# hupe1980/vecgo

Measured on AMD Instinct MI355X. Metric: QPS at recall@10≥0.95, 1M×768 HNSW+PQ; PQ-ADC HBM GB/s vs peak, higher is better.
Workload: dtype f32; 1 GPU; flat_exact_l2_1Mx768_top10 (BASELINE configs[1]): MFMA GEMM nomination + exact re-score + proof; operating_point=flat_exact, rows=1000000, dim=768, k=10, parallelism=1 GPU

## Files before the change

vecgo_amd/csrc/k_flat.hip:

```cpp
#include <algorithm>

#include "vg_device.hpp"
#include "vg_exact.hpp"
#include "vg_cand_replay.hpp"
#include "vg_flat_gemm.hpp"
#include "vg_internal.hpp"
#include "vg_nominate.hpp"
#include "vg_search.hpp"

namespace vg {

struct GemmOperands {
    const float *a, *b;
    int64_t n;
    int dim_words;
    const float *norms;
    bool bf16, dma;
};
struct NomCall {
    hipStream_t st;
    bool dot;
    GemmOperands ops;
    int64_t cnt;
    const uint8_t *mask;
    int64_t mask_stride;
    unsigned ucnt() const { return static_cast<unsigned>(cnt); }
};
struct GemmArgs {
    const NomCall &c;
    const float *queries;
    float *scores = nullptr;
    int tile_stride = 1;
    int64_t out_cols = 0;
    const float *thr = nullptr;
    int thr_stride = 0, thr_off = 0;
    int *counts = nullptr;
    uint64_t *cand = nullptr;
    int cap = 0;
    int cus = 256;
    int *counts_wide = nullptr;
    int skip_stride = 0;
    bool split = false;
    bool screen = false;
    const uint32_t *tile_active = nullptr;

    explicit GemmArgs(const NomCall &call) : c(call), queries(call.ops.a) {}
    static GemmArgs sample(const NomCall &c, float *sc, int stride, int64_t cols)
    {
        GemmArgs a(c);
        a.scores = sc, a.tile_stride = stride, a.out_cols = cols;
        return a;
    }
    static GemmArgs append(const NomCall &c, const float *thr, int sel_k, int *counts, uint64_t *cand, int cap)
    {
        GemmArgs a(c);
        a.thr = thr, a.thr_stride = sel_k, a.thr_off = sel_k - 1, a.counts = counts, a.cand = cand, a.cap = cap;
        return a;
    }
    GemmArgs &wide(int *lines, int compute_units) { return counts_wide = lines, cus = compute_units, *this; }
    GemmArgs &skipping(int stride) { return skip_stride = stride, *this; }
    GemmArgs &split_tile(const uint32_t *image) { return queries = reinterpret_cast<const float *>(image), split = true, *this; }
    GemmArgs &sample_tile(const uint32_t *hi_image) { return split_tile(hi_image); }
    GemmArgs &screen_tile(const uint32_t *hi_image) { return split_tile(hi_image), screen = true, *this; }
    GemmArgs &retry(const uint32_t *active) { return tile_active = active, *this; }
};
constexpr int kCountLine = 32;
static bool gemm_runs_split(bool fused, bool bf16, bool dma, int64_t nq, int dim, int cap, int thr_stride)
{
    return fused && !bf16 && dma && nq > kGemmBM && dim % kGemmBK == 0 && nq * static_cast<int64_t>(cap) < (int64_t(1) << 31) &&
           thr_stride < 65536 && !hook(kHookFlatNoSplit);
}
static float split_gemm_eps(bool dot, int dim)
{
    const float m = static_cast<float>(3 * dim + 16) * 5.9604645e-8f;
    return dot ? 1.5001f * 1.52587890625e-5f + 2.52f * m : 3.0002f * 1.52587890625e-5f + 4.03f * m;
}
static float screen_gemm_eps(bool dot, int dim)
{
    const float m = static_cast<float>(dim + 16) * 5.9604645e-8f;
    return dot ? 0.00390625f + 7.62939453125e-6f + 2.52f * m : 0.0078125f + 1.52587890625e-5f + 4.03f * m;
}
float bf16_filter_eps(bool dot) { return (dot ? 0.00390625f : 0.0078125f) * 1.02f; }
static bool gemm_skips_sample(bool dma, int64_t nq, bool bf16, bool split = false)
{
    if (bf16 || split || hook(kHookFlatRescoreSample)) return false;
    return !(dma && nq <= 3 * kG32BM && !hook(kHookFlatNoSmallTile));
}
__global__ void counts_narrow_kernel(const int *__restrict__ wide, int64_t nq, int *__restrict__ counts)
{
    const int64_t q = static_cast<int64_t>(blockIdx.x) * blockDim.x + threadIdx.x;
    if (q < nq) counts[q] = wide[q * kCountLine];
}

template <class Kern, class... Args>
static int32_t launch_lds(Kern kern, dim3 grid, dim3 threads, size_t lds, hipStream_t st, Args... args)
{
    VG_HIP(hipFuncSetAttribute(reinterpret_cast<const void *>(kern), hipFuncAttributeMaxDynamicSharedMemorySize, static_cast<int>(lds)));
    if (grid.x != 0) VG_LAUNCH(kern, grid, threads, lds, st, args...);
    return VG_OK;
}
template <bool DOT, int M, bool BF16, class F>
static int32_t with_g32_tile(int rb, F f)
{
    constexpr int kMost = BF16 ? 4 : 3;
    if (rb <= 1) return f(flat_gemm_dma32_kernel<DOT, M, 1, BF16>, g32_lds_bytes<1>());
    if (rb == 2) return f(flat_gemm_dma32_kernel<DOT, M, 2, BF16>, g32_lds_bytes<2>());
    if (rb == 3) return f(flat_gemm_dma32_kernel<DOT, M, 3, BF16>, g32_lds_bytes<3>());
    return f(flat_gemm_dma32_kernel<DOT, M, kMost, BF16>, g32_lds_bytes<kMost>());
}

template <bool DOT, int MODE>
static int32_t launch_gemm_t(const GemmArgs &a)
{
    const NomCall &c = a.c;
    const bool dma = c.ops.dma, bf16 = c.ops.bf16;
    const hipStream_t st = c.st;
    const int skip = MODE == 2 ? a.skip_stride : 0;
    VG_CHECK(skip == 0 || (skip > 1 && gemm_skips_sample(dma, c.cnt, bf16, a.split)), VG_ERR_INVALID_ARG, "launch_gemm: skip_stride on a kernel without it");
    const int64_t mt = (c.cnt + kGemmBM - 1) / kGemmBM, nt = (c.ops.n + kGemmBN - 1) / kGemmBN;
    const int64_t tiles = skip ? nt - gemm_skip_sampled_tiles(nt, skip) : (nt + a.tile_stride - 1) / a.tile_stride;
    const dim3 grid(static_cast<unsigned>(mt * ((tiles + 7) / 8) * 8)), threads(kGemmThreads);
    auto big_grid = [&](int64_t bnt ) {
        const int64_t bmt = (c.cnt + kBigBM - 1) / kBigBM;
        const int64_t slots = bmt * ((bnt + 7) / 8) * 8, per_cu = std::max(a.cus / 8, 1) * 8;
        return dim3(static_cast<unsigned>(std::min(slots, per_cu)));
    };
    auto launch_big = [&](auto kern, size_t lds, auto... extra) -> int32_t {
        if (a.counts_wide && !a.tile_active) VG_HIP(hipMemsetAsync(a.counts_wide, 0, sizeof(int) * static_cast<size_t>(c.cnt) * kCountLine, st));
        VG_TRY(launch_lds(kern, big_grid((c.ops.n + kBigBN - 1) / kBigBN), dim3(kBigThreads), lds, st, a.queries, c.cnt, c.ops.b, c.ops.n,
                          c.ops.dim_words, c.ops.norms, a.thr, a.thr_stride, a.thr_off, a.counts_wide ? a.counts_wide : a.counts, a.cand, a.cap, c.mask,
                          c.mask_stride, a.counts_wide ? kCountLine : 1, extra...));
        if (a.counts_wide)
            VG_LAUNCH(counts_narrow_kernel, dim3(static_cast<unsigned>((c.cnt + 255) / 256)), dim3(256), 0, st, a.counts_wide, c.cnt, a.counts);
        return VG_OK;
    };
    auto launch_tile = [&](auto kern, dim3 blocks, size_t lds, auto... last) -> int32_t {
        return launch_lds(kern, blocks, threads, lds, st, a.queries, c.cnt, c.ops.b, c.ops.n, c.ops.dim_words, c.ops.norms, a.scores, a.tile_stride, a.out_cols, a.thr,
                          a.thr_stride, a.thr_off, a.counts, a.cand, a.cap, c.mask, c.mask_stride, last...);
    };
    auto launch_128 = [&](auto kern, size_t lds, int last) { return launch_tile(kern, grid, lds, last); };
    auto launch_g32 = [&](auto kern, size_t lds) { return launch_tile(kern, dim3(static_cast<unsigned>(tiles)), lds); };
    constexpr int M = MODE == 0 ? 1 : MODE;
    const int rb = static_cast<int>((c.cnt + kG32BM - 1) / kG32BM);
    if constexpr (MODE == 1) {
        if (a.split) {
            VG_CHECK(!bf16 && gemm_runs_split(true, false, dma, c.cnt, c.ops.dim_words, 0, 0), VG_ERR_INVALID_ARG, "launch_gemm: sample tile on a call without it");
            return launch_lds(flat_gemm_sample_big_kernel<DOT, 3>, big_grid((tiles + 1) / 2), dim3(kBigThreads), big_lds_bytes<3, true>(), st, a.queries, c.cnt,
                              c.ops.b, c.ops.n, c.ops.dim_words, c.ops.norms, a.scores, a.tile_stride, a.out_cols, c.mask, c.mask_stride);
        }
    }
    if (MODE == 2 && a.split) {
        VG_CHECK(!bf16 && gemm_runs_split(true, false, dma, c.cnt, c.ops.dim_words, a.cap, a.thr_stride), VG_ERR_INVALID_ARG, "launch_gemm: split tile on a call without it");
        if (a.screen) return launch_big(flat_gemm_screen_big_kernel<DOT, 3>, big_lds_bytes<3, true>());
        VG_CHECK(!a.tile_active || (c.cnt <= 32 * kBigBM && a.counts_wide), VG_ERR_INVALID_ARG, "launch_gemm: tile_active is one word, with wide counters");
        note_flat_split_launch();
        return launch_big(flat_gemm_split_big_kernel<DOT, 3>, big_lds_bytes<3>(), a.tile_active);
    }
    if (skip && tiles == 0) return VG_OK;
    if (bf16) {
        if (c.cnt <= 4 * kG32BM && !hook(kHookFlatNoSmallTile)) return with_g32_tile<DOT, M, true>(rb, launch_g32);
        if (MODE == 2 && c.cnt > kGemmBM && c.cnt * static_cast<int64_t>(a.cap) < (int64_t(1) << 31) && a.thr_stride < 65536 &&
            !hook(kHookFlatNoBigTile)) {
            const bool two = hook(kHookFlatBigTile2);
            auto kern = two ? flat_gemm_bf16_big_kernel<DOT, 2> : hook(kHookFlatBigEarlyB) ? flat_gemm_bf16_big_kernel<DOT, 3, 512> : flat_gemm_bf16_big_kernel<DOT, 3>;
            return launch_big(kern, two ? big_lds_bytes<2>() : big_lds_bytes<3>());
        }
        return launch_128(flat_gemm_dma_kernel<DOT, M, 0, true>, kDmaLdsBytes, 0);
    }
    if (dma && MODE != 0 && c.cnt <= 3 * kG32BM && !hook(kHookFlatNoSmallTile)) return with_g32_tile<DOT, M, false>(rb, launch_g32);
    if (dma) return launch_128(flat_gemm_dma_kernel<DOT, MODE>, kDmaLdsBytes, skip);
    return launch_128(flat_gemm_kernel<DOT, MODE>, kGemmLdsBytes, skip);
}

template <int MODE>
static int32_t launch_gemm(const GemmArgs &a)
{
    return a.c.dot ? launch_gemm_t<true, MODE>(a) : launch_gemm_t<false, MODE>(a);
}

__global__ void f32_to_bf16_pad_kernel(const float *__restrict__ src, int64_t rows, int dim, int dim_pad, uint16_t *__restrict__ dst)
{
    const int64_t i = static_cast<int64_t>(blockIdx.x) * blockDim.x + threadIdx.x;
    if (i >= rows * dim_pad) return;
    const int64_t r = i / dim_pad;
    const int j = static_cast<int>(i - r * dim_pad);
    const uint32_t u = j < dim ? __float_as_uint(src[r * dim + j]) : 0u;
    uint16_t v;
    if ((u & 0x7F800000u) == 0x7F800000u && (u & 0x007FFFFFu) != 0)
        v = static_cast<uint16_t>((u >> 16) | 0x0040u);
    else
        v = static_cast<uint16_t>((u + 0x7FFFu + ((u >> 16) & 1u)) >> 16);
    dst[i] = v;
}

static int64_t flat_hi_image_rows(int64_t rows) { return (rows + kBigBM - 1) / kBigBM * kBigBM; }
__global__ void flat_split_queries_kernel(const float *__restrict__ src, int64_t rows, int dim, uint32_t *__restrict__ dst,
                                          uint32_t *__restrict__ hi_dst)
{
    const int64_t i = static_cast<int64_t>(blockIdx.x) * blockDim.x + threadIdx.x;
    const int half = dim / 2;
    const int64_t r = i / half;
    if (r >= (rows + kBigBM - 1) / kBigBM * kBigBM) return;
    const int64_t rs = r < rows ? r : rows - 1;
    const int p = static_cast<int>(i - r * half), s = p >> 4, w = p & 15;
    const float2 v = *reinterpret_cast<const float2 *>(src + rs * dim + 32 * s + 2 * w);
    uint32_t hi, lo;
    split2_bf16(v.x, v.y, hi, lo);
    if (r < rows) {
        dst[r * dim + 32 * s + w] = hi;
        dst[r * dim + 32 * s + 16 + w] = lo;
    }
    const int R = static_cast<int>(r & (kBigBM - 1));
    hi_dst[((r / kBigBM) * (dim / 32) + s) * (kBigBM * 16) + R * 16 + (((w >> 2) ^ ((R >> 2) & 3)) << 2) + (w & 3)] = hi;
}

__global__ __launch_bounds__(256) void flat_todo_kernel(const int *__restrict__ flags, const int *__restrict__ always,
                                                        int cnt, int *__restrict__ todo,
                                                        unsigned long long *__restrict__ stats, const int *__restrict__ counts)
{
    __shared__ int part[256];
    __shared__ unsigned long long appended[256];
    const int tid = threadIdx.x;
    const int per = (cnt + 255) / 256;
    const int lo = tid * per < cnt ? tid * per : cnt, hi = lo + per < cnt ? lo + per : cnt;
    if (!flags) {
        if (tid == 0) atomicAdd(&stats[0], static_cast<unsigned long long>(cnt));
        return;
    }
    const bool all = *always != 0;
    int mine = 0;
    unsigned long long app = 0;
    for (int i = lo; i < hi; i++) {
        mine += (all || flags[i] != 0);
        if (counts) app += static_cast<unsigned long long>(counts[i]);
    }
    part[tid] = mine;
    appended[tid] = app;
    __syncthreads();
    if (tid == 0) {
        int run = 0;
        app = 0;
        for (int t = 0; t < 256; t++) {
            const int c = part[t];
            part[t] = run;
// ... 171 lines not shown
        for (int64_t c = wave; c < chunks; c += kSelWaves) {
            float4 v[4];
#pragma unroll
            for (int u = 0; u < 4; u++) v[u] = row4[c * 256 + u * 64 + lane];
#pragma unroll
            for (int u = 0; u < 4; u++) {
                const int64_t i = a0 + c * 1024 + (u * 64 + lane) * 4;
                const float vals[4] = {v[u].x, v[u].y, v[u].z, v[u].w};
                float mn = fminf(fminf(vals[0], vals[1]), fminf(vals[2], vals[3]));
                if (!__ballot(make_key(mn, 0u, false) < tk.tau)) continue;
#pragma unroll
                for (int e = 0; e < 4; e++)
                    tk.offer(make_key(vals[e], static_cast<uint32_t>(i + e), false), lane);
            }
        }
    }
    {
        const int64_t head_end = (a0 < r1 && a1 > a0) ? a0 : r1;
        for (int64_t i0 = r0 + wave * 64; i0 < head_end; i0 += kSelThreads) {
            const int64_t i = i0 + lane;
            tk.offer(i < head_end ? make_key(row[i], static_cast<uint32_t>(i), false) : kKeyMax, lane);
        }
        const int64_t tail_begin = (a0 < r1 && a1 > a0) ? a1 : r1;
        for (int64_t i0 = tail_begin + wave * 64; i0 < r1; i0 += kSelThreads) {
            const int64_t i = i0 + lane;
            tk.offer(i < r1 ? make_key(row[i], static_cast<uint32_t>(i), false) : kKeyMax, lane);
        }
    }
    wg_rank_merge<kSelWaves>(tk, lists, valid, wave, lane, tid, kc,
                             partial + (q * slices + s) * kc);
}

template <bool DOT>
__global__ __launch_bounds__(256) void flat_verify_kernel(
    const float *__restrict__ base, int64_t n, int dim, const float *__restrict__ queries,
    const float *__restrict__ norms_max , const uint32_t *__restrict__ cand_ids,
    const float *__restrict__ cand_scores, int kc, int k, uint32_t *__restrict__ ids,
    float *__restrict__ scores, int *fallback, const float *__restrict__ thr, int thr_stride,
    int thr_off, const int *__restrict__ counts, int cap, float eps_extra, const int *only)
{
    __shared__ uint64_t keys[64];
    const Sub16 sub = Sub16::make(threadIdx.x);
    const int64_t q = blockIdx.x;
    if (only && only[q] == 0) return;
    const float *qv = queries + q * dim;
    for (int c = threadIdx.x >> 4; c < kc; c += 16) {
        const uint32_t id = cand_ids[q * kc + c];
        uint64_t key = kKeyMax;
        if (id != VG_INVALID_ID) {
            const float v = exact_pair16<DOT, kPair>(base + static_cast<int64_t>(id) * dim, qv, dim, sub);
            key = make_key(v, id, DOT);
        }
        if ((threadIdx.x & 15) == 0) keys[c] = key;
    }
    __syncthreads();
    if (threadIdx.x >= 64) return;
    const int lane = threadIdx.x;
    WaveTopK tk;
    tk.init(k);
    tk.offer(lane < kc ? keys[lane] : kKeyMax, lane);
    float qn = 0.0f;
    for (int j = lane; j < dim; j += 64) qn = __builtin_fmaf(qv[j], qv[j], qn);
    for (int off = 32; off > 0; off >>= 1) qn += __shfl_xor(qn, off);
    const uint64_t kth = readlane_u64(tk.list, k - 1);
    bool ok = true;
    float tau;
    bool have_all;
    if (thr) {
        const float tq = thr[q * thr_stride + thr_off];
        const int cnt = counts[q];
        if (cnt > cap) ok = false;
        tau = cnt > kc ? fminf(tq, cand_scores[q * kc + (kc - 1)]) : tq;
        have_all = (tq == INFINITY) && cnt <= kc;
    } else {
        tau = cand_scores[q * kc + (kc - 1)];
        have_all = (n <= kc);
    }
    if (ok && !have_all) {
        const float xmax = norms_max[0];
        const float eps = (4.0f * (static_cast<float>(dim) * 5.9604645e-8f) + eps_extra) * (qn + xmax) + 1e-30f;
        if (tau == INFINITY) {
            ok = true;
        } else if (kth == kKeyMax) {
            ok = false;
        } else if (DOT) {
            const float dk = key_score(kth, true);
            ok = dk > (-tau) + eps;
        } else {
            const float dk = key_score(kth, false);
            ok = dk < (tau + qn) - eps;
        }
    }
    if (lane < k) {
        const uint64_t e = tk.list;
        ids[q * k + lane] = e == kKeyMax ? VG_INVALID_ID : key_row(e);
        scores[q * k + lane] = e == kKeyMax ? (DOT ? -INFINITY : INFINITY) : key_score(e, DOT);
    }
    if (lane == 0) fallback[q] = ok ? 0 : 1;
}

template <bool DOT>
__global__ __launch_bounds__(256) void flat_verify_all_kernel(
    const float *__restrict__ base, int dim, const float *__restrict__ queries,
    const float *__restrict__ norms_max , const uint64_t *__restrict__ cand, const int *__restrict__ counts,
    int cap, int k, uint32_t *__restrict__ ids, float *__restrict__ scores, int *__restrict__ fallback,
    const float *__restrict__ thr, int thr_stride, int thr_off, float eps_extra)
{
    __shared__ uint64_t lists[4 * 64];
    __shared__ int valid[4];
    __shared__ uint64_t best[64];
    const Sub16 sub = Sub16::make(threadIdx.x);
    const int64_t q = blockIdx.x;
    const int tid = threadIdx.x, lane = tid & 63, wave = tid >> 6;
    const float *qv = queries + q * dim;
    const int total = counts[q];
    const int cnt = total < cap ? total : cap;
    WaveTopK tk;
    tk.init(k);
    for (int c0 = wave * 4; c0 < cnt; c0 += 16) {
        const int c = c0 + (lane >> 4);
        uint64_t key = kKeyMax;
        if (c < cnt) {
            const uint32_t id = key_row(cand[q * cap + c]);
            const float v = exact_pair16<DOT, kPair>(base + static_cast<int64_t>(id) * dim, qv, dim, sub);
            if ((lane & 15) == 0) key = make_key(v, id, DOT);
        }
        tk.offer(key, lane);
    }
    wg_rank_merge<4>(tk, lists, valid, wave, lane, tid, k, best);
    __syncthreads();
    if (tid >= 64) return;
// ... 96 lines not shown
        const uint64_t floor_key = min_keys ? min_keys[q] : 0;
        const uint8_t *mq = mask ? mask + q * mask_stride : nullptr;
        WaveTopK tk;
        tk.init(k);
        for (int64_t i0 = r0 + wave * 4; i0 < r1; i0 += 16) {
            const int64_t i = i0 + (lane >> 4);
            uint64_t key = kKeyMax;
            if (i < r1 && mask_bit(mq, i)) {
                const float v = exact_pair16<DOT, kPair>(base + i * dim, qv, dim, sub);
                if ((lane & 15) == 0) {
                    key = make_key(v, static_cast<uint32_t>(i), DOT);
                    if (min_keys && key <= floor_key) key = kKeyMax;
                }
            }
            tk.offer(key, lane);
        }
        wg_rank_merge<4>(tk, lists, valid, wave, lane, tid, k, out);
        __syncthreads();
    }
}

constexpr int kScanQB = 8;
constexpr int kGemmMaxK = 48;
constexpr int kFlatMaxK = 512;
constexpr int kScreenMaxK = 16;
static bool gemm_runs_screen(bool split, int k)
{
    return split && !hook(kHookFlatNoScreen) && k <= (hook(kHookFlatScreenFail) ? kGemmMaxK : kScreenMaxK);
}
static bool sample_runs_big(bool split, bool use_sample)
{
    return split && use_sample && !hook(kHookFlatF32Sample);
}
constexpr int kScanMaxBatch = 4;
template <bool DOT>
__global__ __launch_bounds__(256) void flat_scan_mq_kernel(const float *__restrict__ base, int64_t n, int dim,
                                                           const float *__restrict__ queries, int nq, int slices,
                                                           int k, uint64_t *__restrict__ partial)
{
    extern __shared__ float qlds[];
    uint64_t *lists = reinterpret_cast<uint64_t *>(qlds + static_cast<size_t>(kScanQB) * dim);
    int *valid = reinterpret_cast<int *>(lists + 4 * 64);
    const int s = blockIdx.x;
    const int tid = threadIdx.x, lane = tid & 63, wave = tid >> 6;
    for (int t = tid; t < nq * dim; t += 256) qlds[t] = queries[t];
    __syncthreads();
    const Sub16 sub = Sub16::make(tid);
    const int nblk = dim >> 6;
    const int64_t r0 = n * s / slices, r1 = n * (s + 1) / slices;
    WaveTopK tk[kScanQB];
#pragma unroll
    for (int qi = 0; qi < kScanQB; qi++) tk[qi].init(k);
    for (int64_t i0 = r0 + wave * 4; i0 < r1; i0 += 16) {
        const int64_t i = i0 + (lane >> 4);
        const bool live = i < r1;
        const float *row = base + (live ? i : r1 - 1) * dim;
        float4 rr[16];
        const float4 *r4 = reinterpret_cast<const float4 *>(row) + sub.f4;
#pragma unroll
        for (int e = 0; e < 16; e++)
            if (e < nblk) rr[e] = load_stream(r4 + e * 16);
#pragma unroll
        for (int qi = 0; qi < kScanQB; qi++) {
            if (qi < nq) {
                const float v = exact_rowregs16<DOT>(rr, nblk, row, qlds + static_cast<size_t>(qi) * dim, dim, sub);
                uint64_t key = kKeyMax;
// ... 107 lines not shown
}
static int32_t sample_thresholds(const NomCall &c, const NomScratch &s, int stride, int sel_k, float *thr, bool sampled, const uint32_t *image = nullptr,
                                 int cus = 0)
{
    if (!sampled) {
        VG_LAUNCH(fill_f32_kernel, dim3(static_cast<unsigned>((c.cnt * sel_k + 255) / 256)), dim3(256), 0, c.st, thr, c.cnt * sel_k, INFINITY);
        return VG_OK;
    }
    GemmArgs a = GemmArgs::sample(c, s.sc, stride, s.cols);
    if (image) a.sample_tile(image).wide(nullptr, cus);
    VG_TRY(launch_gemm<1>(a));
    return select_thresholds(s, c.cnt, sel_k, s.sid, thr, c.st);
}
static int32_t launch_flat_pick(const ProbeNominated &nom, int64_t cnt, const int *only, hipStream_t st)
{
    VG_LAUNCH(flat_pick_kernel, dim3(static_cast<unsigned>(cnt)), dim3(256), 0, st, nom.cand, nom.counts, nom.cap, kFlatKc, nom.cand_id, nom.cand_sc, only);
    return VG_OK;
}
static int32_t launch_flat_verify(bool dot, int k, const vg_index *idx, const float *queries, int64_t cnt, const ProbeNominated &nom,
                                  float eps_extra, uint32_t *ids, float *scores, int *fail, const int *only, hipStream_t st)
{
    return with_metric(dot, [&](auto dot_c) -> int32_t {
        constexpr bool DOT = decltype(dot_c)::value;
        const dim3 grid(static_cast<unsigned>(cnt)), threads(256);
        if (nom.thr && k > 64)
            VG_LAUNCH(flat_verify_sort_kernel<DOT>, grid, threads, sizeof(uint64_t) * static_cast<size_t>(nom.cap), st, idx->d_vectors, idx->dim, queries,
                      idx->d_norm_max, nom.cand, nom.counts, nom.cap, k, ids, scores, fail, nom.thr, nom.sel_k, nom.sel_k - 1, eps_extra);
        else if (nom.thr && k > kGemmMaxK)
            VG_LAUNCH(flat_verify_all_kernel<DOT>, grid, threads, 0, st, idx->d_vectors, idx->dim, queries, idx->d_norm_max, nom.cand, nom.counts,
                      nom.cap, k, ids, scores, fail, nom.thr, nom.sel_k, nom.sel_k - 1, eps_extra);
        else
            VG_LAUNCH(flat_verify_kernel<DOT>, grid, threads, 0, st, idx->d_vectors, idx->n, idx->dim, queries, idx->d_norm_max, nom.cand_id,
                      nom.cand_sc, kFlatKc, k, ids, scores, fail, nom.thr, nom.sel_k, nom.sel_k - 1, nom.counts, nom.cap, eps_extra, only);
        return VG_OK;
    });
}

struct FlatCall {
    vg_index *idx;
    int k;
    hipStream_t st;
    bool dot;
    const float *q;
    int64_t nq;
    const uint8_t *mask;
    int64_t mask_stride;
    uint32_t *oid;
    float *osc;
    int64_t n = idx->n;
    int dim = idx->dim;
    FlatCall range(int64_t q0, int64_t cnt) const
    {
        FlatCall r = *this;
        r.q += q0 * dim, r.nq = cnt, r.oid += q0 * k, r.osc += q0 * k;
        if (mask) r.mask += q0 * mask_stride;
        return r;
    }
    NomCall nom() const { return {st, dot, fp32_operands(idx, q, !hook(kHookFlatNoDma)), nq, mask, mask_stride}; }
};
constexpr int kFlatCap = 4096;
constexpr int kFlatSampleStride = 64;
static int exact_slices(int64_t n) { return static_cast<int>(std::min<int64_t>(256, std::max<int64_t>(1, n / 64))); }
struct FlatScratch : NomScratch {
    bool fused;
    bool use_sample;
    bool bf16;
// ... 74 lines not shown
    int *flags = ar.get<int>(i_flags), *todo = ar.get<int>(i_todo);
    uint64_t *fpartial = ar.get<uint64_t>(i_fpartial);
    VG_HIP(hipMemsetAsync(flags, 0, sizeof(int) * static_cast<size_t>(qc), call.st));
    VG_HIP(hipMemsetAsync(flags + qc, 1, sizeof(int), call.st));
    for (int64_t q0 = 0; q0 < call.nq; q0 += qc) {
        const FlatCall c = call.range(q0, std::min(qc, call.nq - q0));
        VG_TRY(launch_flat_todo(flags, flags + qc, static_cast<int>(c.nq), todo, c.idx->d_flat_stats, c.st));
        VG_TRY(launch_flat_exact(c, todo, ex_slices, c.k, fpartial, nullptr));
        VG_TRY(launch_topk_merge(fpartial, c.nq, ex_slices, c.k, c.dot, c.oid, c.osc, c.st));
    }
    return VG_OK;
}

static int32_t flat_unfused_chunk(const FlatCall &c, const FlatScratch &s)
{
    const NomCall nc = c.nom();
    {
        ProfScope prof(c.idx->ctx, "flat_gemm", c.st);
        VG_TRY(launch_gemm<0>(GemmArgs::sample(nc, s.sc, 1, c.n)));
    }
    {
        ProfScope prof(c.idx->ctx, "flat_select", c.st);
        VG_TRY(launch_flat_select(s, c.nq, kFlatKc, c.st));
    }
    VG_TRY(launch_topk_merge(s.partial, c.nq, s.slices, kFlatKc, false, s.nom.cand_id, s.nom.cand_sc, c.st));
    ProbeNominated nom = s.nom;
    nom.thr = nullptr;
    return launch_flat_verify(c.dot, c.k, c.idx, c.q, c.nq, nom, 0.0f, c.oid, c.osc, s.flags, nullptr, c.st);
}

static int32_t flat_screen_retry(const FlatCall &c, const NomCall &nc, const FlatScratch &s)
{
    const ProbeNominated &nom = s.nom;
    VG_LAUNCH(flat_retry_prepare_kernel, dim3(1), dim3(kBigBM), 0, c.st, s.flags, hook(kHookFlatScreenFail), static_cast<int>(c.nq), nom.thr,
              nom.sel_k, nom.sel_k - 1, nom.counts, s.counts_wide, s.tile_active, c.idx->d_flat_stats);
    {
        ProfScope prof(c.idx->ctx, "flat_retry", c.st);
        VG_TRY(launch_gemm<2>(GemmArgs::append(nc, nom.thr, nom.sel_k, nom.counts, nom.cand, nom.cap)
                                  .wide(s.counts_wide, c.idx->ctx->compute_units)
                                  .split_tile(reinterpret_cast<const uint32_t *>(s.qbf))
                                  .retry(s.tile_active)));
    }
    VG_TRY(launch_flat_pick(nom, c.nq, s.flags, c.st));
    return launch_flat_verify(c.dot, c.k, c.idx, c.q, c.nq, nom, split_gemm_eps(c.dot, c.dim), c.oid, c.osc, s.flags, s.flags, c.st);
}

static int32_t flat_fused_chunk(const FlatCall &c, const FlatScratch &s)
{
    const vg_index *idx = c.idx;
    const ProbeNominated &nom = s.nom;
    NomCall nc = c.nom();
    const bool split = gemm_runs_split(true, s.bf16, nc.ops.dma, c.nq, c.dim, nom.cap, nom.sel_k);
    const bool screen = gemm_runs_screen(split, c.k);
    const float eps_extra = screen ? screen_gemm_eps(c.dot, c.dim) : split ? split_gemm_eps(c.dot, c.dim) : s.bf16 ? bf16_filter_eps(c.dot) : 0.0f;
    if (s.bf16) VG_TRY(gemm_operands(c.q, c.nq, c.dim, c.n, idx->d_norms, idx->d_vectors_bf16, idx->vectors_bf16_dim, s.qbf, c.st, &nc.ops));
    if (split)
        VG_LAUNCH(flat_split_queries_kernel, dim3(static_cast<unsigned>((flat_hi_image_rows(c.nq) * (c.dim / 2) + 255) / 256)), dim3(256), 0, c.st, c.q,
                  c.nq, c.dim, reinterpret_cast<uint32_t *>(s.qbf), s.qhi);
    VG_TRY(sample_thresholds(nc, s, kFlatSampleStride, nom.sel_k, nom.thr, s.use_sample, sample_runs_big(split, s.use_sample) ? s.qhi : nullptr,
                             idx->ctx->compute_units));
    if (s.bf16 || split) VG_LAUNCH(flat_thr_cap_kernel, dim3(nc.ucnt()), dim3(64), 0, c.st, nom.thr, nom.sel_k, c.q, c.dim, idx->d_norm_max);
    const bool once = s.use_sample && gemm_skips_sample(nc.ops.dma, c.nq, s.bf16, split);
    if (!once) VG_HIP(hipMemsetAsync(nom.counts, 0, sizeof(int) * static_cast<size_t>(c.nq), c.st));
    {
        ProfScope prof(idx->ctx, "flat_gemm", c.st);
        if (once)
            VG_LAUNCH(flat_sample_append_kernel, dim3(nc.ucnt()), dim3(kSampleAppendThreads), 0, c.st, s.sc, s.cols, kFlatSampleStride, nom.thr,
                      nom.sel_k, nom.sel_k - 1, nom.counts, nom.cand, nom.cap);
        GemmArgs a = GemmArgs::append(nc, nom.thr, nom.sel_k, nom.counts, nom.cand, nom.cap);
        a.wide(s.bf16 || split ? s.counts_wide : nullptr, idx->ctx->compute_units).skipping(once ? kFlatSampleStride : 0);
        if (screen)
            a.screen_tile(s.qhi);
        else if (split)
            a.split_tile(reinterpret_cast<const uint32_t *>(s.qbf));
        VG_TRY(launch_gemm<2>(a));
    }
    if (c.k <= kGemmMaxK) VG_TRY(launch_flat_pick(nom, c.nq, nullptr, c.st));
    VG_TRY(launch_flat_verify(c.dot, c.k, idx, c.q, c.nq, nom, eps_extra, c.oid, c.osc, s.flags, nullptr, c.st));
    return screen ? flat_screen_retry(c, nc, s) : VG_OK;
}

static void flat_debug_counts(const FlatCall &c, int64_t q0, const FlatScratch &s)
{
    std::vector<int> hf(c.nq), hc(c.nq);
    (void)hipMemcpyAsync(hf.data(), s.flags, sizeof(int) * c.nq, hipMemcpyDeviceToHost, c.st);
    (void)hipMemcpyAsync(hc.data(), s.nom.counts, sizeof(int) * c.nq, hipMemcpyDeviceToHost, c.st);
    (void)hipStreamSynchronize(c.st);
    int64_t nf = 0, csum = 0, cmax = 0;
    for (int f : hf) nf += f != 0;
    for (int n : hc) { csum += n; cmax = std::max<int64_t>(cmax, n); }
    fprintf(stderr, "[vg_search_flat] chunk q0=%lld cnt=%lld: %lld queries failed the proof; "
            "appended candidates avg %.1f max %lld\n", (long long)q0, (long long)c.nq, (long long)nf,
            s.fused ? double(csum) / c.nq : 0.0, (long long)(s.fused ? cmax : 0));
}

static int32_t flat_fallback_pages(const FlatCall &c, const FlatScratch &s)
{
    const int *always = s.flags + s.qc;
    const dim3 grid(static_cast<unsigned>(c.nq));
    for (int off = 0; off < c.k; off += 64) {
        const int kk = std::min(64, c.k - off);
        VG_TRY(launch_flat_exact(c, s.todo, s.ex_slices, kk, s.fpartial, off ? s.min_keys : nullptr));
        VG_TRY(launch_topk_merge(s.fpartial, c.nq, s.ex_slices, kk, c.dot, s.fid, s.fsc, c.st, s.flags, always));
        if (c.k <= 64)
            VG_LAUNCH(flat_patch_kernel, grid, dim3(64), 0, c.st, s.flags, always, c.k, s.fid, s.fsc, c.oid, c.osc);
        else
            VG_LAUNCH(flat_page_patch_kernel, grid, dim3(64), 0, c.st, s.flags, always, c.k, off, kk, c.dot, s.fid, s.fsc, c.oid, c.osc, s.min_keys);
    }
    return VG_OK;
}

// ... 298 lines not shown
```

vecgo_amd/csrc/vg_api.hip:

```cpp
#include "vg_internal.hpp"

namespace vg {

static thread_local std::string g_last_error;

void set_error(const char *fmt, ...)
{
    char buf[512];
    va_list ap;
    va_start(ap, fmt);
    vsnprintf(buf, sizeof buf, fmt, ap);
    va_end(ap);
    g_last_error = buf;
}

bool is_device_ptr(const void *p)
{
    if (!p) return false;
    hipPointerAttribute_t a;
    hipError_t e = hipPointerGetAttributes(&a, p);
    (void)hipGetLastError();
    if (e != hipSuccess) return false;
    return a.type == hipMemoryTypeDevice || a.type == hipMemoryTypeManaged;
}
// ... 266 lines not shown
    if (idx->d_flat_stats) (void)hipFree(idx->d_flat_stats);
    if (idx->d_vectors_bf16) (void)hipFree(idx->d_vectors_bf16);
    if (idx->d_rq_tiles) (void)hipFree(idx->d_rq_tiles);
    if (idx->d_rq_norms) (void)hipFree(idx->d_rq_norms);
    for (uint32_t **a : {&idx->d_hnsw_l0, &idx->d_hnsw_slot, &idx->d_hnsw_adj}) vg::drop_device(a);
    for (float **a : {&idx->d_hnsw_l0_dist, &idx->d_hnsw_l0_cdist, &idx->d_hnsw_adj_cdist}) vg::drop_device(a);
    vg::drop_device(&idx->d_hnsw_tomb);
    vg::drop_device(&idx->d_hnsw_level_off);
    if (idx->d_vamana) (void)hipFree(idx->d_vamana);
    if (idx->d_pq_rows) (void)hipFree(idx->d_pq_rows);
    if (idx->d_rq_rows) (void)hipFree(idx->d_rq_rows);
    if (idx->d_sq_tiles) (void)hipFree(idx->d_sq_tiles);
    (void)vg::nom_free(idx->sq_nom, idx->ctx->stream);
    (void)vg::nom_free(idx->pq_nom, idx->ctx->stream);
    if (idx->d_int4_rows) (void)hipFree(idx->d_int4_rows);
    if (idx->d_centroids) (void)hipFree(idx->d_centroids);
    if (idx->d_part_off) (void)hipFree(idx->d_part_off);
    delete idx;
    return VG_OK;
}

#include <atomic>
namespace vg {
static std::atomic<int> g_hooks[kHookCount];
static std::once_flag g_hooks_once;
static const char *const kHookNames[kHookCount] = {"VG_FLAT_NO_SMALL_TILE", "VG_FLAT_UNFUSED", "VG_FLAT_NO_SCAN",
                                                   "VG_FLAT_FORCE_EXACT", "VG_FLAT_NO_DMA", "VG_FLAT_DEBUG",
                                                   "VG_PROBE_NO_GROUP", "VG_ADC_BIGK_EXHAUSTIVE", "VG_BUILD_DEBUG",
                                                   "VG_KM_NO_MFMA", "VG_KM_LIST_ALL", "VG_KM_BF16", "VG_KM_NO_BF16", "VG_BRUTE_NO_FLAT", "VG_PQ_NO_MFMA",
                                                   "VG_PQ_LIST_ALL", "VG_PQ_FP32_MFMA", "VG_PROBE_NO_GEMM", "VG_FLAT_NO_BIG_TILE",
                                                   "VG_FLAT_BIG_TILE_2", "VG_FLAT_BIG_EARLY_B", "VG_PQ_NOM_ALWAYS", "VG_KM_NO_RANGES", "VG_NO_CAND_REPLAY",
                                                   "VG_VAMANA_SMALL_SCRATCH", "VG_FLAT_RESCORE_SAMPLE", "VG_PTHR_FORCE_HIST",
                                                   "VG_WALK_SMALL_SCRATCH", "VG_FLAT_NO_SPLIT", "VG_FLAT_NO_SCREEN", "VG_FLAT_SCREEN_FAIL",
                                                   "VG_FLAT_F32_SAMPLE", "VG_PREFILTER_SMALL_SCRATCH"};
static void hooks_from_env()
{
    for (int h = 0; h < kHookCount; h++) {
        const char *e = getenv(kHookNames[h]);
        g_hooks[h].store(e && e[0] == '1' ? 1 : 0, std::memory_order_relaxed);
    }
}
bool hook(Hook h)
{
    std::call_once(g_hooks_once, hooks_from_env);
    return g_hooks[h].load(std::memory_order_relaxed) != 0;
}
}

VG_API int32_t vg_debug_set_hook(const char *name, int32_t on)
{
    VG_CHECK(name, VG_ERR_INVALID_ARG, "vg_debug_set_hook: NULL name");
    std::call_once(vg::g_hooks_once, vg::hooks_from_env);
    for (int h = 0; h < vg::kHookCount; h++)
        if (std::strcmp(name, vg::kHookNames[h]) == 0) {
            vg::g_hooks[h].store(on ? 1 : 0, std::memory_order_relaxed);
            return VG_OK;
        }
    vg::set_error("vg_debug_set_hook: unknown hook %s", name);
    return VG_ERR_INVALID_ARG;
}
```

vecgo_amd/csrc/vg_internal.hpp:

```cpp
#pragma once

#include <hip/hip_runtime.h>

#include <algorithm>
#include <atomic>
#include <cstdarg>
#include <cstdint>
#include <cstdio>
#include <cstdlib>
#include <cstring>
#include <mutex>
#include <string>
#include <vector>

#include "../../include/vecgo_hip.h"

struct vg_index;

#define VG_API extern "C" __attribute__((visibility("default")))

namespace vg {

void set_error(const char *fmt, ...);

// ... 40 lines not shown
    kHookFlatNoSmallTile,
    kHookFlatUnfused,
    kHookFlatNoScan,
    kHookFlatForceExact,
    kHookFlatNoDma,
    kHookFlatDebug,
    kHookProbeNoGroup,
    kHookAdcBigkExhaustive,
    kHookBuildDebug,
    kHookKmNoMfma,
    kHookKmListAll,
    kHookKmBf16,
    kHookKmNoBf16,
    kHookBruteNoFlat,
    kHookPqNoMfma,
    kHookPqListAll,
    kHookPqFp32Mfma,
    kHookProbeNoGemm,
    kHookFlatNoBigTile,
    kHookFlatBigTile2,
    kHookFlatBigEarlyB,
    kHookPqNomAlways,
    kHookKmNoRanges,
    kHookNoCandReplay,
    kHookVamanaSmallScratch,
    kHookFlatRescoreSample,
    kHookPthrForceHist,
    kHookWalkSmallScratch,
    kHookFlatNoSplit,
    kHookFlatNoScreen,
    kHookFlatScreenFail,
    kHookFlatF32Sample,
    kHookPrefilterSmallScratch,
    kHookCount
};
bool hook(Hook h);

int32_t scratch_alloc(void **out, size_t bytes, hipStream_t s);
int32_t append_row_norms(vg_index *idx, int64_t from, int64_t to, hipStream_t st);
int32_t append_bf16_rows(vg_index *idx, int64_t from, int64_t to, hipStream_t st);
void scratch_free(void *p);
void scratch_trim(int device);

}

struct vg_prof_record {
    const char *name;
    hipEvent_t start, stop;
};

struct vg_arena {
    char *base = nullptr;
    size_t cap = 0;
};

struct vg_ctx {
    int device = 0;
    std::mutex arena_mu;
    std::vector<std::pair<hipStream_t, vg_arena>> arenas;
    hipStream_t stream = nullptr;
    int compute_units = 0;
    int64_t hbm_bytes = 0;
    char arch[64] = {0};
    bool profiling = false;
    std::mutex prof_mu;
    std::vector<vg_prof_record> prof;
// ... 373 lines not shown
```

Before: 509,200 queries/s.

## Fuse candidate pick, exact verify and retry-prepare into one kernel

Adds a flat_pick_verify kernel that merges each query's appended candidates into a top-64 list, re-scores them exactly and runs the proof in one launch. This replaces the separate pick, verify and retry-prepare kernels. The wide per-line counters are zeroed inside the query-split kernel instead of by a memset, and the narrowing kernel is skipped because the fused kernel reads the wide counters directly. The aim is to remove several small launches and memsets plus an intermediate candidate round-trip, at the cost of a larger per-query workgroup kernel and more complex counter state handling.

Result: no change. 510,400 queries/s, median of 3 (+0.2%).

```diff
diff --git a/vecgo_amd/csrc/k_flat.hip b/vecgo_amd/csrc/k_flat.hip
--- a/vecgo_amd/csrc/k_flat.hip
+++ b/vecgo_amd/csrc/k_flat.hip
@@ -39,6 +39,7 @@
     int cap = 0;
     int cus = 256;
     int *counts_wide = nullptr;
+    bool wide_zeroed = false, wide_stays = false;
     int skip_stride = 0;
     bool split = false;
     bool screen = false;
@@ -58,6 +59,7 @@
         return a;
     }
     GemmArgs &wide(int *lines, int compute_units) { return counts_wide = lines, cus = compute_units, *this; }
+    GemmArgs &wide_kept(bool zeroed, bool stays) { return wide_zeroed = zeroed, wide_stays = stays, *this; }
     GemmArgs &skipping(int stride) { return skip_stride = stride, *this; }
     GemmArgs &split_tile(const uint32_t *image) { return queries = reinterpret_cast<const float *>(image), split = true, *this; }
     GemmArgs &sample_tile(const uint32_t *hi_image) { return split_tile(hi_image); }
@@ -69,6 +71,10 @@
 {
     return fused && !bf16 && dma && nq > kGemmBM && dim % kGemmBK == 0 && nq * static_cast<int64_t>(cap) < (int64_t(1) << 31) &&
            thr_stride < 65536 && !hook(kHookFlatNoSplit);
+}
+static bool gemm_runs_big_bf16(int64_t nq, int cap, int thr_stride)
+{
+    return nq > kGemmBM && nq * static_cast<int64_t>(cap) < (int64_t(1) << 31) && thr_stride < 65536 && !hook(kHookFlatNoBigTile);
 }
 static float split_gemm_eps(bool dot, int dim)
 {
@@ -126,11 +132,11 @@
         return dim3(static_cast<unsigned>(std::min(slots, per_cu)));
     };
     auto launch_big = [&](auto kern, size_t lds, auto... extra) -> int32_t {
-        if (a.counts_wide && !a.tile_active) VG_HIP(hipMemsetAsync(a.counts_wide, 0, sizeof(int) * static_cast<size_t>(c.cnt) * kCountLine, st));
+        if (a.counts_wide && !a.tile_active && !a.wide_zeroed) VG_HIP(hipMemsetAsync(a.counts_wide, 0, sizeof(int) * static_cast<size_t>(c.cnt) * kCountLine, st));
         VG_TRY(launch_lds(kern, big_grid((c.ops.n + kBigBN - 1) / kBigBN), dim3(kBigThreads), lds, st, a.queries, c.cnt, c.ops.b, c.ops.n,
                           c.ops.dim_words, c.ops.norms, a.thr, a.thr_stride, a.thr_off, a.counts_wide ? a.counts_wide : a.counts, a.cand, a.cap, c.mask,
                           c.mask_stride, a.counts_wide ? kCountLine : 1, extra...));
-        if (a.counts_wide)
+        if (a.counts_wide && !a.wide_stays)
             VG_LAUNCH(counts_narrow_kernel, dim3(static_cast<unsigned>((c.cnt + 255) / 256)), dim3(256), 0, st, a.counts_wide, c.cnt, a.counts);
         return VG_OK;
     };
@@ -159,8 +165,7 @@
     if (skip && tiles == 0) return VG_OK;
     if (bf16) {
         if (c.cnt <= 4 * kG32BM && !hook(kHookFlatNoSmallTile)) return with_g32_tile<DOT, M, true>(rb, launch_g32);
-        if (MODE == 2 && c.cnt > kGemmBM && c.cnt * static_cast<int64_t>(a.cap) < (int64_t(1) << 31) && a.thr_stride < 65536 &&
-            !hook(kHookFlatNoBigTile)) {
+        if (MODE == 2 && gemm_runs_big_bf16(c.cnt, a.cap, a.thr_stride)) {
             const bool two = hook(kHookFlatBigTile2);
             auto kern = two ? flat_gemm_bf16_big_kernel<DOT, 2> : hook(kHookFlatBigEarlyB) ? flat_gemm_bf16_big_kernel<DOT, 3, 512> : flat_gemm_bf16_big_kernel<DOT, 3>;
             return launch_big(kern, two ? big_lds_bytes<2>() : big_lds_bytes<3>());
@@ -195,7 +200,7 @@
 
 static int64_t flat_hi_image_rows(int64_t rows) { return (rows + kBigBM - 1) / kBigBM * kBigBM; }
 __global__ void flat_split_queries_kernel(const float *__restrict__ src, int64_t rows, int dim, uint32_t *__restrict__ dst,
-                                          uint32_t *__restrict__ hi_dst)
+                                          uint32_t *__restrict__ hi_dst, int *__restrict__ counts_wide, uint32_t *__restrict__ tile_active)
 {
     const int64_t i = static_cast<int64_t>(blockIdx.x) * blockDim.x + threadIdx.x;
     const int half = dim / 2;
@@ -209,7 +214,9 @@
     if (r < rows) {
         dst[r * dim + 32 * s + w] = hi;
         dst[r * dim + 32 * s + 16 + w] = lo;
-    }
+        if (p == 0) counts_wide[r * kCountLine] = 0;
+    }
+    if (i == 0) *tile_active = 0u;
     const int R = static_cast<int>(r & (kBigBM - 1));
     hi_dst[((r / kBigBM) * (dim / 32) + s) * (kBigBM * 16) + R * 16 + (((w >> 2) ^ ((R >> 2) & 3)) << 2) + (w & 3)] = hi;
 }
@@ -447,30 +454,10 @@
 }
 
 template <bool DOT>
-__global__ __launch_bounds__(256) void flat_verify_kernel(
-    const float *__restrict__ base, int64_t n, int dim, const float *__restrict__ queries,
-    const float *__restrict__ norms_max , const uint32_t *__restrict__ cand_ids,
-    const float *__restrict__ cand_scores, int kc, int k, uint32_t *__restrict__ ids,
-    float *__restrict__ scores, int *fallback, const float *__restrict__ thr, int thr_stride,
-    int thr_off, const int *__restrict__ counts, int cap, float eps_extra, const int *only)
-{
-    __shared__ uint64_t keys[64];
-    const Sub16 sub = Sub16::make(threadIdx.x);
-    const int64_t q = blockIdx.x;
-    if (only && only[q] == 0) return;
-    const float *qv = queries + q * dim;
-    for (int c = threadIdx.x >> 4; c < kc; c += 16) {
-        const uint32_t id = cand_ids[q * kc + c];
-        uint64_t key = kKeyMax;
-        if (id != VG_INVALID_ID) {
-            const float v = exact_pair16<DOT, kPair>(base + static_cast<int64_t>(id) * dim, qv, dim, sub);
-            key = make_key(v, id, DOT);
-        }
-        if ((threadIdx.x & 15) == 0) keys[c] = key;
-    }
-    __syncthreads();
-    if (threadIdx.x >= 64) return;
-    const int lane = threadIdx.x;
+__device__ __forceinline__ bool flat_prove(const uint64_t *keys, int kc, int k, const float *__restrict__ qv, int dim,
+                                           const float *__restrict__ norms_max, bool fused, float tq, int cnt, int cap, float last_sc,
+                                           bool have_all_rows, float eps_extra, uint32_t *__restrict__ ids, float *__restrict__ scores, int lane)
+{
     WaveTopK tk;
     tk.init(k);
     tk.offer(lane < kc ? keys[lane] : kKeyMax, lane);
@@ -481,15 +468,13 @@
     bool ok = true;
     float tau;
     bool have_all;
-    if (thr) {
-        const float tq = thr[q * thr_stride + thr_off];
-        const int cnt = counts[q];
+    if (fused) {
         if (cnt > cap) ok = false;
-        tau = cnt > kc ? fminf(tq, cand_scores[q * kc + (kc - 1)]) : tq;
+        tau = cnt > kc ? fminf(tq, last_sc) : tq;
         have_all = (tq == INFINITY) && cnt <= kc;
     } else {
-        tau = cand_scores[q * kc + (kc - 1)];
-        have_all = (n <= kc);
+        tau = last_sc;
+        have_all = have_all_rows;
     }
     if (ok && !have_all) {
         const float xmax = norms_max[0];
@@ -508,10 +493,103 @@
     }
     if (lane < k) {
         const uint64_t e = tk.list;
-        ids[q * k + lane] = e == kKeyMax ? VG_INVALID_ID : key_row(e);
-        scores[q * k + lane] = e == kKeyMax ? (DOT ? -INFINITY : INFINITY) : key_score(e, DOT);
-    }
-    if (lane == 0) fallback[q] = ok ? 0 : 1;
+        ids[lane] = e == kKeyMax ? VG_INVALID_ID : key_row(e);
+        scores[lane] = e == kKeyMax ? (DOT ? -INFINITY : INFINITY) : key_score(e, DOT);
+    }
+    return ok;
+}
+
+template <bool DOT>
+__global__ __launch_bounds__(256) void flat_verify_kernel(
+    const float *__restrict__ base, int64_t n, int dim, const float *__restrict__ queries,
+    const float *__restrict__ norms_max , const uint32_t *__restrict__ cand_ids,
+    const float *__restrict__ cand_scores, int kc, int k, uint32_t *__restrict__ ids,
+    float *__restrict__ scores, int *fallback, const float *__restrict__ thr, int thr_stride,
+    int thr_off, const int *__restrict__ counts, int cap, float eps_extra, const int *only)
+{
+    __shared__ uint64_t keys[64];
+    const Sub16 sub = Sub16::make(threadIdx.x);
+    const int64_t q = blockIdx.x;
+    if (only && only[q] == 0) return;
+    const float *qv = queries + q * dim;
+    for (int c = threadIdx.x >> 4; c < kc; c += 16) {
+        const uint32_t id = cand_ids[q * kc + c];
+        uint64_t key = kKeyMax;
+        if (id != VG_INVALID_ID) {
+            const float v = exact_pair16<DOT, kPair>(base + static_cast<int64_t>(id) * dim, qv, dim, sub);
+            key = make_key(v, id, DOT);
+        }
+        if ((threadIdx.x & 15) == 0) keys[c] = key;
+    }
+    __syncthreads();
+    if (threadIdx.x >= 64) return;
+    float tq = 0.0f;
+    int cnt = 0;
+    if (thr) {
+        tq = thr[q * thr_stride + thr_off];
+        cnt = counts[q];
+    }
+    const bool ok = flat_prove<DOT>(keys, kc, k, qv, dim, norms_max, thr != nullptr, tq, cnt, cap, cand_scores[q * kc + (kc - 1)], n <= kc, eps_extra,
+                                    ids + q * k, scores + q * k, static_cast<int>(threadIdx.x));
+    if (threadIdx.x == 0) fallback[q] = ok ? 0 : 1;
+}
+
+template <bool DOT>
+__global__ __launch_bounds__(256) void flat_pick_verify_kernel(
+    const float *__restrict__ base, int dim, const float *__restrict__ queries, const float *__restrict__ norms_max ,
+    const uint64_t *__restrict__ cand, int *__restrict__ counts, int *__restrict__ counts_wide, int cap, int k, uint32_t *__restrict__ ids,
+    float *__restrict__ scores, int *fallback, float *__restrict__ thr, int thr_stride, int thr_off, float eps_extra, const int *only, bool prepare,
+    bool fail_all, uint32_t *__restrict__ tile_active, unsigned long long *__restrict__ stats)
+{
+    constexpr int kc = 64;
+    __shared__ uint64_t lists[4 * 64];
+    __shared__ int valid[4];
+    __shared__ uint64_t best[kc];
+    __shared__ uint64_t keys[kc];
+    const int64_t q = blockIdx.x;
+    if (only && only[q] == 0) return;
+    const int tid = threadIdx.x, lane = tid & 63, wave = tid >> 6;
+    const int cnt = counts_wide ? counts_wide[q * kCountLine] : counts[q];
+    const int c = cnt > cap ? cap : cnt;
+    const uint64_t *src = cand + q * cap;
+    WaveTopK tk;
+    tk.init(kc);
+    for (int i0 = wave * 64; i0 < c; i0 += 256) {
+        const int i = i0 + lane;
+        tk.offer(i < c ? src[i] : kKeyMax, lane);
+    }
+    wg_rank_merge<4>(tk, lists, valid, wave, lane, tid, kc, best);
+    __syncthreads();
+    const Sub16 sub = Sub16::make(threadIdx.x);
+    const float *qv = queries + q * dim;
+    for (int i = tid >> 4; i < kc; i += 16) {
+        const uint64_t e = best[i];
+        uint64_t key = kKeyMax;
+        if (e != kKeyMax) {
+            const uint32_t id = key_row(e);
+            const float v = exact_pair16<DOT, kPair>(base + static_cast<int64_t>(id) * dim, qv, dim, sub);
+            key = make_key(v, id, DOT);
+        }
+        if ((tid & 15) == 0) keys[i] = key;
+    }
+    __syncthreads();
+    if (tid >= 64) return;
+    const uint64_t last = best[kc - 1];
+    const float tq = thr[q * thr_stride + thr_off];
+    const bool ok = flat_prove<DOT>(keys, kc, k, qv, dim, norms_max, true, tq, cnt, cap, last == kKeyMax ? INFINITY : key_score(last, false), false,
+                                    eps_extra, ids + q * k, scores + q * k, lane);
+    if (lane != 0) return;
+    const bool retry = prepare && (fail_all || !ok);
+    fallback[q] = (ok && !retry) ? 0 : 1;
+    if (counts_wide) counts[q] = retry ? 0 : cnt;
+    if (!prepare) return;
+    if (retry) {
+        counts_wide[q * kCountLine] = 0;
+        atomicOr(tile_active, 1u << (q / kBigBM));
+        atomicAdd(&stats[2], 1ull);
+    } else {
+        thr[q * thr_stride + thr_off] = -INFINITY;
+    }
 }
 
 template <bool DOT>
@@ -674,6 +752,7 @@
 {
     return split && use_sample && !hook(kHookFlatF32Sample);
 }
+static bool flat_pick_fused(int k) { return k <= kGemmMaxK && !hook(kHookFlatSplitPick); }
 constexpr int kScanMaxBatch = 4;
 template <bool DOT>
 __global__ __launch_bounds__(256) void flat_scan_mq_kernel(const float *__restrict__ base, int64_t n, int dim,
@@ -847,6 +926,18 @@
         else
             VG_LAUNCH(flat_verify_kernel<DOT>, grid, threads, 0, st, idx->d_vectors, idx->n, idx->dim, queries, idx->d_norm_max, nom.cand_id,
                       nom.cand_sc, kFlatKc, k, ids, scores, fail, nom.thr, nom.sel_k, nom.sel_k - 1, nom.counts, nom.cap, eps_extra, only);
+        return VG_OK;
+    });
+}
+static int32_t launch_flat_pick_verify(bool dot, int k, const vg_index *idx, const float *queries, int64_t cnt, const ProbeNominated &nom, int *counts_wide,
+                                       float eps_extra, uint32_t *ids, float *scores, int *fail, const int *only, uint32_t *tile_active, bool screen_fail,
+                                       hipStream_t st)
+{
+    VG_CHECK(k <= kGemmMaxK && nom.thr && (!tile_active || counts_wide), VG_ERR_INVALID_ARG, "launch_flat_pick_verify: not the 64-candidate regime");
+    return with_metric(dot, [&](auto dot_c) -> int32_t {
+        VG_LAUNCH(flat_pick_verify_kernel<decltype(dot_c)::value>, dim3(static_cast<unsigned>(cnt)), dim3(256), 0, st, idx->d_vectors, idx->dim, queries,
+                  idx->d_norm_max, nom.cand, nom.counts, counts_wide, nom.cap, k, ids, scores, fail, nom.thr, nom.sel_k, nom.sel_k - 1, eps_extra, only,
+                  tile_active != nullptr, screen_fail, tile_active, idx->d_flat_stats);
         return VG_OK;
     });
 }
@@ -987,15 +1078,21 @@
 static int32_t flat_screen_retry(const FlatCall &c, const NomCall &nc, const FlatScratch &s)
 {
     const ProbeNominated &nom = s.nom;
-    VG_LAUNCH(flat_retry_prepare_kernel, dim3(1), dim3(kBigBM), 0, c.st, s.flags, hook(kHookFlatScreenFail), static_cast<int>(c.nq), nom.thr,
-              nom.sel_k, nom.sel_k - 1, nom.counts, s.counts_wide, s.tile_active, c.idx->d_flat_stats);
+    const bool fuse_pick = flat_pick_fused(c.k);
+    if (!fuse_pick)
+        VG_LAUNCH(flat_retry_prepare_kernel, dim3(1), dim3(kBigBM), 0, c.st, s.flags, hook(kHookFlatScreenFail), static_cast<int>(c.nq), nom.thr,
+                  nom.sel_k, nom.sel_k - 1, nom.counts, s.counts_wide, s.tile_active, c.idx->d_flat_stats);
     {
         ProfScope prof(c.idx->ctx, "flat_retry", c.st);
         VG_TRY(launch_gemm<2>(GemmArgs::append(nc, nom.thr, nom.sel_k, nom.counts, nom.cand, nom.cap)
                                   .wide(s.counts_wide, c.idx->ctx->compute_units)
+                                  .wide_kept(true, fuse_pick)
                                   .split_tile(reinterpret_cast<const uint32_t *>(s.qbf))
                                   .retry(s.tile_active)));
     }
+    if (fuse_pick)
+        return launch_flat_pick_verify(c.dot, c.k, c.idx, c.q, c.nq, nom, s.counts_wide, split_gemm_eps(c.dot, c.dim), c.oid, c.osc, s.flags, s.flags, nullptr,
+                                       false, c.st);
     VG_TRY(launch_flat_pick(nom, c.nq, s.flags, c.st));
     return launch_flat_verify(c.dot, c.k, c.idx, c.q, c.nq, nom, split_gemm_eps(c.dot, c.dim), c.oid, c.osc, s.flags, s.flags, c.st);
 }
@@ -1011,27 +1108,34 @@
     if (s.bf16) VG_TRY(gemm_operands(c.q, c.nq, c.dim, c.n, idx->d_norms, idx->d_vectors_bf16, idx->vectors_bf16_dim, s.qbf, c.st, &nc.ops));
     if (split)
         VG_LAUNCH(flat_split_queries_kernel, dim3(static_cast<unsigned>((flat_hi_image_rows(c.nq) * (c.dim / 2) + 255) / 256)), dim3(256), 0, c.st, c.q,
-                  c.nq, c.dim, reinterpret_cast<uint32_t *>(s.qbf), s.qhi);
+                  c.nq, c.dim, reinterpret_cast<uint32_t *>(s.qbf), s.qhi, s.counts_wide, s.tile_active);
     VG_TRY(sample_thresholds(nc, s, kFlatSampleStride, nom.sel_k, nom.thr, s.use_sample, sample_runs_big(split, s.use_sample) ? s.qhi : nullptr,
                              idx->ctx->compute_units));
     if (s.bf16 || split) VG_LAUNCH(flat_thr_cap_kernel, dim3(nc.ucnt()), dim3(64), 0, c.st, nom.thr, nom.sel_k, c.q, c.dim, idx->d_norm_max);
     const bool once = s.use_sample && gemm_skips_sample(nc.ops.dma, c.nq, s.bf16, split);
-    if (!once) VG_HIP(hipMemsetAsync(nom.counts, 0, sizeof(int) * static_cast<size_t>(c.nq), c.st));
+    int *const wide = split || (s.bf16 && gemm_runs_big_bf16(c.nq, nom.cap, nom.sel_k)) ? s.counts_wide : nullptr;
+    const bool fuse_pick = flat_pick_fused(c.k);
+    if (!once && !wide) VG_HIP(hipMemsetAsync(nom.counts, 0, sizeof(int) * static_cast<size_t>(c.nq), c.st));
     {
         ProfScope prof(idx->ctx, "flat_gemm", c.st);
         if (once)
             VG_LAUNCH(flat_sample_append_kernel, dim3(nc.ucnt()), dim3(kSampleAppendThreads), 0, c.st, s.sc, s.cols, kFlatSampleStride, nom.thr,
                       nom.sel_k, nom.sel_k - 1, nom.counts, nom.cand, nom.cap);
         GemmArgs a = GemmArgs::append(nc, nom.thr, nom.sel_k, nom.counts, nom.cand, nom.cap);
-        a.wide(s.bf16 || split ? s.counts_wide : nullptr, idx->ctx->compute_units).skipping(once ? kFlatSampleStride : 0);
+        a.wide(wide, idx->ctx->compute_units).wide_kept(split, fuse_pick).skipping(once ? kFlatSampleStride : 0);
         if (screen)
             a.screen_tile(s.qhi);
         else if (split)
             a.split_tile(reinterpret_cast<const uint32_t *>(s.qbf));
         VG_TRY(launch_gemm<2>(a));
     }
-    if (c.k <= kGemmMaxK) VG_TRY(launch_flat_pick(nom, c.nq, nullptr, c.st));
-    VG_TRY(launch_flat_verify(c.dot, c.k, idx, c.q, c.nq, nom, eps_extra, c.oid, c.osc, s.flags, nullptr, c.st));
+    if (fuse_pick) {
+        VG_TRY(launch_flat_pick_verify(c.dot, c.k, idx, c.q, c.nq, nom, wide, eps_extra, c.oid, c.osc, s.flags, nullptr, screen ? s.tile_active : nullptr,
+                                       hook(kHookFlatScreenFail), c.st));
+    } else {
+        if (c.k <= kGemmMaxK) VG_TRY(launch_flat_pick(nom, c.nq, nullptr, c.st));
+        VG_TRY(launch_flat_verify(c.dot, c.k, idx, c.q, c.nq, nom, eps_extra, c.oid, c.osc, s.flags, nullptr, c.st));
+    }
     return screen ? flat_screen_retry(c, nc, s) : VG_OK;
 }
 
diff --git a/vecgo_amd/csrc/vg_api.hip b/vecgo_amd/csrc/vg_api.hip
--- a/vecgo_amd/csrc/vg_api.hip
+++ b/vecgo_amd/csrc/vg_api.hip
@@ -322,7 +322,7 @@
                                                    "VG_FLAT_BIG_TILE_2", "VG_FLAT_BIG_EARLY_B", "VG_PQ_NOM_ALWAYS", "VG_KM_NO_RANGES", "VG_NO_CAND_REPLAY",
                                                    "VG_VAMANA_SMALL_SCRATCH", "VG_FLAT_RESCORE_SAMPLE", "VG_PTHR_FORCE_HIST",
                                                    "VG_WALK_SMALL_SCRATCH", "VG_FLAT_NO_SPLIT", "VG_FLAT_NO_SCREEN", "VG_FLAT_SCREEN_FAIL",
-                                                   "VG_FLAT_F32_SAMPLE", "VG_PREFILTER_SMALL_SCRATCH"};
+                                                   "VG_FLAT_F32_SAMPLE", "VG_PREFILTER_SMALL_SCRATCH", "VG_FLAT_SPLIT_PICK"};
 static void hooks_from_env()
 {
     for (int h = 0; h < kHookCount; h++) {
diff --git a/vecgo_amd/csrc/vg_internal.hpp b/vecgo_amd/csrc/vg_internal.hpp
--- a/vecgo_amd/csrc/vg_internal.hpp
+++ b/vecgo_amd/csrc/vg_internal.hpp
@@ -96,6 +96,7 @@
     kHookFlatScreenFail,
     kHookFlatF32Sample,
     kHookPrefilterSmallScratch,
+    kHookFlatSplitPick,
     kHookCount
 };
 bool hook(Hook h);
```
